# johanngerberding/voxelnet-pytorch

Hardware: AMD Instinct MI355X
Metric: point-clouds/sec fwd+bwd, KITTI car voxel grid, batch=2 (higher is better)
Workload: dtype bf16; 1 GPU; KITTI car config (voxel 0.2x0.2x0.4 m, grid 10x400x352, T=35), batch=2 per GPU, fwd+bwd train step (BASELINE configs[1]); global_batch=2, points_per_frame=19861, parallelism=dp1, launch_mode=eager+native-executor+one-call-step

## Files before the change

### include/voxelnet_hip.h

```cpp
#ifndef VOXELNET_HIP_H
#define VOXELNET_HIP_H

#include <stddef.h>
#include <stdint.h>

#ifdef __cplusplus
extern "C" {
#endif

#define VN_OK 0
#define VN_EINVAL (-1)
#define VN_EUNSUPPORTED (-2)
#define VN_EWORKSPACE (-3)

typedef enum { VN_F32 = 0, VN_BF16 = 1,
               VN_F32X3 = 2,
               VN_F32X3S = 3 } vnDtype;

typedef void *vnStream;

int vn_abi_version(void);
const char *vn_build_info(void);
const char *vn_build_id(void);

typedef struct {
    int32_t D, H, W;
    float vz, vy, vx;
    float ox, oy, oz;
    int32_t T;
} vnGrid;

size_t vn_voxelize_workspace_bytes(int64_t n_points, const vnGrid *grid);

int vn_voxelize_index(const float *points , int64_t n_points,
                      const vnGrid *grid, void *workspace, size_t workspace_bytes,
                      int32_t *k_out, vnStream stream);

int vn_voxelize_gather(const float *points, int64_t n_points, const vnGrid *grid,
                       void *workspace, size_t workspace_bytes, int64_t K,
                       int64_t batch_index, int32_t coord_cols,
                       float *feature , int64_t *coord ,
                       int64_t *number , const int32_t *k_dev, vnStream stream);

size_t vn_voxelize_host_workspace_bytes(int64_t n_points, const vnGrid *grid);
int vn_voxelize_host_index(const float *points , int64_t n_points, const vnGrid *grid,
                           void *workspace , size_t workspace_bytes, int64_t *k_out);
int vn_voxelize_host_gather(const float *points, int64_t n_points, const vnGrid *grid, const void *workspace,
                            size_t workspace_bytes, int64_t K, int64_t batch_index, int32_t coord_cols,
                            float *feature , int64_t *coord ,
                            int64_t *number );

typedef struct {
    const float *w1, *b1, *g1, *be1; float *rm1, *rv1;
    const float *w2, *b2, *g2, *be2; float *rm2, *rv2;
} vnVfeWeights;
typedef struct {
    float *dw1, *db1, *dg1, *dbe1, *dw2, *db2, *dg2, *dbe2;
} vnVfeGrads;

size_t vn_vfe_workspace_bytes(int64_t K, int32_t T);
int vn_vfe_fwd(const float *feature , int64_t K, int32_t T, const vnVfeWeights *w,
               int32_t training, float momentum, float eps, float *voxelwise ,
               float *stats , void *workspace, size_t workspace_bytes, vnStream stream);
int vn_vfe_fwd_rows(const float *feature, int64_t K, int32_t T, const vnVfeWeights *w, int32_t training, float momentum,
                    float eps, float *voxelwise, void *rows_bf16, float *stats, void *workspace, size_t workspace_bytes,
                    vnStream stream);
int vn_vfe_bwd(const float *feature, int64_t K, int32_t T, const vnVfeWeights *w, const float *stats,
               const float *d_voxelwise, const vnVfeGrads *g, void *workspace,
               size_t workspace_bytes, int32_t workspace_is_forwards, vnStream stream);

size_t vn_vfe_layer_workspace_bytes(int64_t K, int32_t T, int32_t cin, int32_t units);
int vn_vfe_layer_fwd(const float *inputs , const uint8_t *mask , int64_t K, int32_t T,
                     int32_t cin, int32_t units, const float *weight, const float *bias, const float *gamma,
                     const float *beta, float *running_mean, float *running_var, int32_t training, float momentum,
                     float eps, float *out , void *workspace, size_t workspace_bytes, vnStream stream);
int vn_vfe_layer_bwd(const float *inputs, const uint8_t *mask, const float *d_out , int64_t K,
                     int32_t T, int32_t cin, int32_t units, const float *weight, int32_t training, float *d_inputs,
                     float *d_weight, float *d_bias, float *d_gamma, float *d_beta, void *workspace,
                     size_t workspace_bytes, vnStream stream);

int vn_scatter_dense_fwd(const float *voxelwise , const int64_t *coord ,
                         int64_t K, int32_t C, int32_t B, int32_t D, int32_t H, int32_t W,
                         void *dense, vnDtype dense_dtype, int32_t dense_channels,
                         int32_t split, vnStream stream);
int vn_scatter_dense_update(const float *voxelwise , const int64_t *coord, int64_t K,
                            int32_t C, int32_t B, int32_t D, int32_t H, int32_t W, void *dense,
                            vnDtype dense_dtype, int32_t dense_channels, int32_t split, vnStream stream);

int vn_scatter_dense_bwd(const void *d_dense, vnDtype dtype, const int64_t *coord,
                         int64_t K, int32_t C, int32_t B, int32_t D, int32_t H, int32_t W,
                         float *d_voxelwise , vnStream stream);

typedef struct {
    int32_t dtype;
    int32_t B;
    int32_t Ds, Hs, Ws;
    int32_t Dr, Hr, Wr;
    int32_t Cs;
    int32_t src_wrap;
    int32_t Cr;
    int32_t kD, kH, kW;
    int32_t mulD, mulH, mulW;
    int32_t tmulD, tmulH, tmulW;
    int32_t padD, padH, padW;
    int32_t divD, divH, divW;
    int64_t src_sB, src_sD, src_sH, src_sW;
    int64_t out_sB, out_sD, out_sH, out_sW;
} vnConv;

int64_t vn_conv_stats_slab_rows(const vnConv *geom);
int vn_conv_gather_gemm(const void *src, const void *w_packed ,
                        const float *bias , void *out, vnDtype out_dtype,
                        const vnConv *geom, int32_t accumulate, float *stats_slab,
                        vnStream stream);
int32_t vn_conv_plan_id(const vnConv *geom);

size_t vn_conv_wgrad_workspace_bytes(const vnConv *geom, int32_t split, int64_t n_rows);
int vn_conv_wgrad(const void *src , const void *rows , float *dw_packed,
                  const vnConv *geom, int32_t split, void *workspace, size_t workspace_bytes,
                  vnStream stream);
int32_t vn_conv_wgrad_plan_id(const vnConv *geom, int32_t split, int64_t n_rows);
int vn_conv_wgrad_partials(const void *src, const void *rows, const vnConv *geom, int32_t split,
                           const int64_t *row_list, int64_t n_rows, void *workspace,
                           size_t workspace_bytes, int32_t *chunks, vnStream stream);
int vn_conv_wgrad_partials_split_pass(const void *src, const void *rows, const vnConv *geom, int32_t pass, void *workspace,
                                      size_t workspace_bytes, int32_t *chunks, vnStream stream);

int vn_conv_dgrad_bn_bwd(const void *src, const void *w_packed, void *out, vnDtype out_dtype, const vnConv *geom,
                         const void *bn_y, vnDtype bn_y_dtype, const float *bn_stats, float *slab, vnStream stream);
int vn_conv_gather_gemm_rows(const void *src, const void *w_packed, const float *bias, void *out,
                             vnDtype out_dtype, const vnConv *geom, const int64_t *row_list,
                             int64_t row_cap, const int32_t *row_count, int32_t out_linear,
                             float *stats_slab, vnStream stream);
int vn_conv_wgrad_rows(const void *src, const void *rows, float *dw_packed, const vnConv *geom,
                       const int64_t *row_list, int64_t n_rows, void *workspace, size_t workspace_bytes,
                       vnStream stream);
int vn_conv_wgrad_partials_counted(const void *src, const void *rows, const vnConv *geom, const int64_t *row_list,
                                   int64_t row_cap, const int32_t *row_count, void *workspace, size_t workspace_bytes,
                                   int32_t *chunks, vnStream stream);
size_t vn_active_sites_workspace_bytes(const vnConv *geom);
int vn_active_sites(const int64_t *coord, int64_t K, const vnConv *geom, void *workspace,
                    size_t workspace_bytes, int64_t *list, int64_t cap, int32_t *count, vnStream stream);
int vn_voxel_index_grid(const int64_t *coord, int64_t K, int32_t B, int32_t D, int32_t H, int32_t W,
                        int32_t *grid , vnStream stream);
int64_t vn_rulebook_slab_rows(int64_t cap);
int vn_rulebook_combine(const float *P, const int32_t *index_grid, const int64_t *list, int64_t cap,
                        const int32_t *count, const vnConv *geom, const float *bias, void *y,
                        vnDtype y_dtype, float *stats_slab, vnStream stream);
int vn_fill_rows(void *y, vnDtype dtype, int64_t M, int32_t C, int64_t stride, const float *values,
// ... 487 lines not shown
```

### voxelnet-pytorch_amd/csrc/vfe.hip

```cpp
#include "common.h"

namespace {

constexpr int C1 = 16, C2 = 64, CIN = 7;
constexpr int ST1 = 0, ST2 = 4 * C1;
constexpr int STATS_FLOATS = 4 * C1 + 4 * C2;
constexpr int TS = 65;
constexpr int NW = 2, NT = NW * 64;
constexpr int VFE_BLOCKS_MAX = 1024;
constexpr int V_AGG1 = 0, V_AM1 = 16, V_DAG1 = 32;
template <bool B2> constexpr int sv_u() { return B2 ? 48 : 16; }
template <bool B2> constexpr int sv_stride() { return B2 ? 113 : 81; }
constexpr int V_U = sv_u<true>(), V_S = V_U, SV = sv_stride<true>();
constexpr int SLAB_P1 = 64, SLAB_P2 = 2 * C2, SLAB_B1 = 2 * C2;
constexpr int SLAB_B2 = C2 + C2 * 32 + 64;
constexpr int SLAB_B3 = 128;

#ifdef VFE_TRACE
__device__ unsigned long long *g_vfe_trace;
__device__ int g_vfe_trace_kernel;
__shared__ int vfe_tr_item_s[8];
__shared__ int vfe_tr_on;
#define VFE_TR_KERNEL(id)                                                                                              \
    if (threadIdx.x == 0) vfe_tr_on = g_vfe_trace != nullptr && g_vfe_trace_kernel == (id);                            \
// ... 365 lines not shown
constexpr int PART_CHUNK = 4096;

constexpr int NCLS = 4;
__device__ __forceinline__ void classify16(const uint4 &q, int64_t v0, int64_t K, int c[NCLS]) {
    const uint32_t w[4] = {q.x, q.y, q.z, q.w};
#pragma unroll
    for (int j = 0; j < 16; ++j) {
        const int r = (w[j >> 2] >> (8 * (j & 3))) & 255;
        const bool in = v0 + j < K;
        c[0] += in && r <= 8; c[1] += in && r > 8 && r <= 16; c[2] += in && r > 16 && r <= 32; c[3] += in && r > 32;
    }
}

__global__ void __launch_bounds__(256) k_vfe_partition(const uint8_t *__restrict__ rows, int64_t K, int32_t *__restrict__ list,
                                                       int32_t *__restrict__ counts) {
    VN_PRIO_MAIN();
    __shared__ int red[4][3 * NCLS];
    const int tid = threadIdx.x, lane = tid & 63, wave = tid >> 6;
    const int64_t n16 = (K + 15) >> 4, mine = (int64_t)blockIdx.x * (PART_CHUNK / 16);
    int before[NCLS] = {0, 0, 0, 0}, total[NCLS] = {0, 0, 0, 0};
    for (int64_t i = tid; i < n16; i += 256) {
        int c[NCLS] = {0, 0, 0, 0};
        classify16(*reinterpret_cast<const uint4 *>(rows + i * 16), i * 16, K, c);
#pragma unroll
        for (int k = 0; k < NCLS; ++k) { total[k] += c[k]; before[k] += i < mine ? c[k] : 0; }
    }
    const int64_t v0 = (mine + tid) * 16;
    int c[NCLS] = {0, 0, 0, 0};
    uint4 q = make_uint4(0, 0, 0, 0);
    if (v0 < K) {
        q = *reinterpret_cast<const uint4 *>(rows + v0);
        classify16(q, v0, K, c);
    }
    int inc[NCLS];
#pragma unroll
    for (int k = 0; k < NCLS; ++k) {
        int x = c[k], t = total[k], bf = before[k];
#pragma unroll
        for (int o = 1; o < 64; o <<= 1) {
            const int y = __shfl_up(x, o, 64);
            if (lane >= o) x += y;
            t += __shfl_xor(t, o, 64);
            bf += __shfl_xor(bf, o, 64);
        }
        inc[k] = x;
        if (lane == 63) red[wave][k] = x;
        if (lane == 0) { red[wave][NCLS + k] = t; red[wave][2 * NCLS + k] = bf; }
    }
    __syncthreads();
    int pos[NCLS], tot[NCLS];
#pragma unroll
    for (int k = 0; k < NCLS; ++k) {
        int base = 0, t = 0, bf = 0;
        for (int w = 0; w < 4; ++w) {
            if (w < wave) base += red[w][k];
            t += red[w][NCLS + k];
            bf += red[w][2 * NCLS + k];
        }
        tot[k] = t;
        pos[k] = bf + base + inc[k] - c[k];
    }
    pos[1] += tot[0];
    pos[2] += tot[0] + tot[1];
    pos[3] += tot[0] + tot[1] + tot[2];
    if (v0 < K) {
        const uint32_t w[4] = {q.x, q.y, q.z, q.w};
#pragma unroll
        for (int j = 0; j < 16; ++j) {
            const int r = (w[j >> 2] >> (8 * (j & 3))) & 255;
            if (v0 + j < K) {
                if (r <= 8) list[pos[0]++] = (int32_t)(v0 + j);
                else if (r <= 16) list[pos[1]++] = (int32_t)(v0 + j);
                else if (r <= 32) list[pos[2]++] = (int32_t)(v0 + j);
                else list[pos[3]++] = (int32_t)(v0 + j);
            }
        }
    }
    if (blockIdx.x == 0 && tid == 0) { counts[0] = tot[0]; counts[1] = tot[1]; counts[2] = tot[2]; counts[3] = tot[3]; }
}

template <int G>
__device__ __forceinline__ void p2_item(const float *__restrict__ feature, int T, const WorkList &wk, int first, int n,
                                        int item, const float *wl, const float *stats, const WaveLds &L, int lane,
                                        const FwdRegs &F, float &s1, float &s2) {
    int v, r, s, j; float wgt;
    item_lane<G>(wk, first, n, item, T, lane, v, r, s, j, wgt);
    float x[CIN], m, h1[C1], p1[C1];
    load_row(feature, v, T, j, j < r, x, m);
    forward_to_h2<G, false, false>(wl, stats, L, lane, v, r, s, j, x, m, F, h1, p1);
    L.mk[lane] = wgt;
    __builtin_amdgcn_wave_barrier();
    for (int t = 0; t < 64; ++t) {
        const float h = L.tile[t * TS + lane], wh = L.mk[t] * h;
        s1 += wh;
        s2 = fmaf(wh, h, s2);
    }
    __builtin_amdgcn_wave_barrier();
}

__global__ void __launch_bounds__(NT) __attribute__((amdgpu_waves_per_eu(2, 2))) k_vfe_p2(const float *__restrict__ feature, int T, VfeParams P, WorkList wk,
                                               const float *__restrict__ stats, float *__restrict__ slabs) {
    VN_PRIO_MAIN();
    extern __shared__ __attribute__((aligned(16))) float smem[];
    const int lane = threadIdx.x & 63, wave = threadIdx.x >> 6;
    VFE_TR_KERNEL(2)
    float *wl = smem;
    load_weights_lds(P, wl, smem + WL_SIZE);
    const WaveLds L = carve_lds<false>(smem + WL_SIZE, wave);
    const Items it = load_items(wk);
    FwdRegs F;
    load_fwd_regs(P, smem + WL_SIZE, lane, F);
    __syncthreads();
    float s1 = 0.f, s2 = 0.f;
#define BODY_P2(G, first, n, item) p2_item<G>(feature, T, wk, first, n, item, wl, stats, L, lane, F, s1, s2);
    VFE_FOR_ITEMS(it, BODY_P2)
#undef BODY_P2
    __syncthreads();
    float vals[2] = {s1, s2};
    slab_write(smem, vals, 2, lane, wave, slabs + (size_t)blockIdx.x * SLAB_P2);
}

template <int G>
__device__ __forceinline__ void p3_item(const float *__restrict__ feature, int T, const WorkList &wk, int first, int n,
                                        int item, const float *wl, const float *stats, const WaveLds &L, int lane,
                                        const FwdRegs &F, float mean2, float S2, float be2,
                                        float *__restrict__ voxelwise, bf16_t *__restrict__ rows16) {
    constexpr int R = 64 / G;
    int v, r, s, j; float wgt;
    item_lane<G>(wk, first, n, item, T, lane, v, r, s, j, wgt);
    float x[CIN], m, h1[C1], p1[C1];
    load_row(feature, v, T, j, j < r, x, m);
    forward_to_h2<G, false, false>(wl, stats, L, lane, v, r, s, j, x, m, F, h1, p1);
    for (int ts = 0; ts < G; ++ts) {
        const int tv = uni(L.sid[ts]), tr = uni(L.sid[8 + ts]);
        if (tv < 0) continue;
        float agg = -INFINITY, vlo = -INFINITY, anym = 0.f, allm = 1.f;
        for (int t = 0; t < tr; ++t) {
            const float p = fmaf(S2, L.tile[(ts * R + t) * TS + lane] - mean2, be2);
            const float mk = L.mk[ts * R + t];
            agg = fmaxf(agg, p);
            vlo = fmaxf(vlo, p * mk);
            anym = fmaxf(anym, mk);
            allm = fminf(allm, mk);
        }
        float vhi = agg * anym;
        if (anym != allm) vhi = fmaxf(agg, 0.f);
        voxelwise[(int64_t)tv * 128 + lane] = vlo;
        voxelwise[(int64_t)tv * 128 + 64 + lane] = vhi;
        if (rows16) {
            rows16[(int64_t)tv * 128 + lane] = (bf16_t)vlo;
            rows16[(int64_t)tv * 128 + 64 + lane] = (bf16_t)vhi;
        }
    }
    __builtin_amdgcn_wave_barrier();
}

__global__ void __launch_bounds__(NT) __attribute__((amdgpu_waves_per_eu(2, 2))) k_vfe_p3(const float *__restrict__ feature, int T, VfeParams P, WorkList wk,
                                               const float *__restrict__ stats, float *__restrict__ voxelwise,
                                               bf16_t *__restrict__ rows16) {
    VN_PRIO_MAIN();
    extern __shared__ __attribute__((aligned(16))) float smem[];
    const int lane = threadIdx.x & 63, wave = threadIdx.x >> 6;
    VFE_TR_KERNEL(3)
    float *wl = smem;
    load_weights_lds(P, wl, smem + WL_SIZE);
    const WaveLds L = carve_lds<false>(smem + WL_SIZE, wave);
    const Items it = load_items(wk);
    FwdRegs F;
    load_fwd_regs(P, smem + WL_SIZE, lane, F);
    __syncthreads();
    const float mean2 = stats[ST2 + lane], S2 = stats[ST2 + 2 * C2 + lane], be2 = stats[ST2 + 3 * C2 + lane];
#define BODY_P3(G, first, n, item) p3_item<G>(feature, T, wk, first, n, item, wl, stats, L, lane, F, mean2, S2, be2, voxelwise, rows16);
    VFE_FOR_ITEMS(it, BODY_P3)
#undef BODY_P3
}

__device__ __forceinline__ void slab_pair_sum(const float *__restrict__ slabs, int nslabs, int stride, int off, int C,
                                              int c, double &o1, double &o2) {
    __shared__ double r1[4], r2[4];
    double s1 = 0.0, s2 = 0.0;
    for (int b = threadIdx.x; b < nslabs; b += 256) {
        s1 += slabs[(size_t)b * stride + off + c];
        s2 += slabs[(size_t)b * stride + off + C + c];
    }
#pragma unroll
    for (int o = 32; o > 0; o >>= 1) {
        s1 += __shfl_xor(s1, o, 64);
        s2 += __shfl_xor(s2, o, 64);
    }
    if ((threadIdx.x & 63) == 0) { r1[threadIdx.x >> 6] = s1; r2[threadIdx.x >> 6] = s2; }
    __syncthreads();
    o1 = (r1[0] + r1[1]) + (r1[2] + r1[3]);
    o2 = (r2[0] + r2[1]) + (r2[2] + r2[3]);
}

__global__ void __launch_bounds__(256) k_vfe_finalize(const float *__restrict__ slabs, int nslabs, int slab_stride, int C,
                                                      int64_t rows,
                                                      const float *__restrict__ gamma, const float *__restrict__ beta,
                                                      float *running_mean, float *running_var, int training,
                                                      float momentum, float eps, float *__restrict__ st) {
    VN_PRIO_MAIN();
    const int c = blockIdx.x;
    double mean, var;
    float p_gamma = 0.f, p_beta = 0.f, p_rm = 0.f, p_rv = 0.f;
    if (threadIdx.x == 0) { p_gamma = gamma[c]; p_beta = beta[c]; p_rm = running_mean[c]; p_rv = running_var[c]; }
    if (training) {
        double s1, s2;
        slab_pair_sum(slabs, nslabs, slab_stride, 0, C, c, s1, s2);
        const double n = (double)rows;
        mean = s1 / n;
        var = s2 / n - mean * mean;
        if (var < 0.0) var = 0.0;
        if (threadIdx.x == 0) {
            running_mean[c] = (float)((1.0 - momentum) * p_rm + momentum * mean);
            const double unb = n > 1.0 ? var * n / (n - 1.0) : var;
            running_var[c] = (float)((1.0 - momentum) * p_rv + momentum * unb);
        }
    } else {
        mean = p_rm;
        var = p_rv;
    }
    if (threadIdx.x == 0) {
        const float invstd = (float)(1.0 / sqrt(var + (double)eps));
        st[c] = (float)mean;
        st[C + c] = invstd;
        st[2 * C + c] = p_gamma * invstd;
        st[3 * C + c] = p_beta;
    }
}

template <int R>
__device__ __forceinline__ void impulses(const WaveLds &L, int row0, int tr, int lane, float mean2, float S2, float be2,
                                         float dlo, float dhi, int &r1, float &g1, int &r2, float &g2, float &xh1,
                                         float &xh2, float inv2) {
    float agg = -INFINITY, vlo = -INFINITY;
    r1 = 0; r2 = 0;
    float h_r1 = 0.f, h_r2 = 0.f, mk_r1 = 0.f;
#pragma unroll
    for (int t0 = 0; t0 < R; t0 += 8) {
        if (R > 16 && t0 >= tr) break;
        float h[8];
#pragma unroll
        for (int u = 0; u < 8; ++u) h[u] = L.tile[(row0 + t0 + u) * TS + lane];
        const f32x4_t ma = *reinterpret_cast<const f32x4_t *>(L.mk + row0 + t0), mb = *reinterpret_cast<const f32x4_t *>(L.mk + row0 + t0 + 4);
        const float mk[8] = {ma[0], ma[1], ma[2], ma[3], mb[0], mb[1], mb[2], mb[3]};
#pragma unroll
        for (int u = 0; u < 8; ++u) {
            const int t = t0 + u;
            const float p = fmaf(S2, h[u] - mean2, be2);
            const float pm = p * mk[u];
            const bool c2 = t < tr && p > agg, c1 = t < tr && pm > vlo;
            agg = c2 ? p : agg; r2 = c2 ? t : r2; h_r2 = c2 ? h[u] : h_r2;
            vlo = c1 ? pm : vlo; r1 = c1 ? t : r1; h_r1 = c1 ? h[u] : h_r1; mk_r1 = c1 ? mk[u] : mk_r1;
        }
    }
    float best = -INFINITY, mk_ap = 0.f;
#pragma unroll
// ... 288 lines not shown
    const int lane = threadIdx.x & 63, wave = threadIdx.x >> 6;
    VFE_TR_KERNEL(-1)
    const Items it = load_items(wk);
    float acc[C1 * CIN + C1];
#pragma unroll
    for (int e = 0; e < C1 * CIN + C1; ++e) acc[e] = 0.f;
#define BODY_B3(G, first, n, item)                                                                                   \
    {                                                                                                                \
        int v, r, s, j; float wgt;                                                                                   \
        item_lane<G>(wk, first, n, item, T, lane, v, r, s, j, wgt);                                                  \
        const bool active = j < r;                                                                                   \
        float x[CIN], m, h1[C1];                                                                                     \
        load_row(feature, v, T, j, active, x, m);                                                                    \
        layer1(P, x, h1);                                                                                            \
        if (active) {                                                                                                \
            const float *src = dp1_ws + ((int64_t)v * T + j) * C1;                                                   \
            _Pragma("unroll") for (int i = 0; i < C1; i += 4) {                                                      \
                const float4 d = *reinterpret_cast<const float4 *>(src + i);                                         \
                const float dd[4] = {d.x, d.y, d.z, d.w};                                                            \
                _Pragma("unroll") for (int q = 0; q < 4; ++q) {                                                      \
                    const int o = i + q;                                                                             \
                    const float dh = fmaf(coef1[o], dd[q], wgt * fmaf(coef1[C1 + o], h1[o] - stats[ST1 + o], coef1[2 * C1 + o])); \
                    const float da = h1[o] > 0.f ? dh : 0.f;                                                         \
                    acc[C1 * CIN + o] += da;                                                                         \
                    _Pragma("unroll") for (int k = 0; k < CIN; ++k) acc[o * CIN + k] = fmaf(da, x[k], acc[o * CIN + k]); \
                }                                                                                                    \
            }                                                                                                        \
        }                                                                                                            \
    }
    VFE_FOR_ITEMS(it, BODY_B3)
#undef BODY_B3
    lane_sums_to_slab(acc, smem, lane, wave, slabs + (size_t)blockIdx.x * SLAB_B3);
}

struct ReduceJobs {
    const float *slabs[4];
    float *out[4];
    int stride[4], off[4], n[4], first[5], nslabs[4];
};
constexpr int RED_E = 16, RED_G = 64;
__global__ void __launch_bounds__(RED_E * RED_G) k_vfe_reduce_multi(const ReduceJobs J) {
    VN_PRIO_MAIN();
    int j = 0;
#pragma unroll
    for (int q = 1; q < 4; ++q)
        if ((int)blockIdx.x >= J.first[q]) j = q;
    const float *slabs = J.slabs[0];
    float *out = J.out[0];
    int stride = J.stride[0], off = J.off[0], n = J.n[0], first = J.first[0], nslabs = J.nslabs[0];
#pragma unroll
    for (int q = 1; q < 4; ++q)
        if (j == q) {
            slabs = J.slabs[q]; out = J.out[q]; stride = J.stride[q]; off = J.off[q]; n = J.n[q]; first = J.first[q];
            nslabs = J.nslabs[q];
        }
    __shared__ double red[RED_G][RED_E + 1];
    const int e = threadIdx.x & (RED_E - 1), g = threadIdx.x / RED_E;
    const int i = ((int)blockIdx.x - first) * RED_E + e;
    double s = 0.0;
    if (i < n) {
        for (int b0 = g; b0 < nslabs; b0 += RED_G * 16) {
            float x[16];
#pragma unroll
            for (int u = 0; u < 16; ++u) {
                const int b = b0 + RED_G * u;
                x[u] = b < nslabs ? slabs[(size_t)b * stride + off + i] : 0.f;
            }
#pragma unroll
            for (int u = 0; u < 16; ++u) s += x[u];
        }
    }
    red[g][e] = s;
    __syncthreads();
    if (threadIdx.x < RED_E && i < n) {
        double t = 0.0;
        for (int q = 0; q < RED_G; ++q) t += red[q][threadIdx.x];
        out[i] = (float)t;
    }
}

struct Plan {
    int blocks, blocks_b2;
    size_t lds_small, lds_full, lds_b2;
    size_t off_slabs, off_slabs3, off_coef, off_rows, off_list, off_counts, off_dp1, bytes;
};

Plan make_plan(int64_t K, int T) {
    Plan p{};
    int64_t b = vn_ceil_div(K, 2 * NW);
    if (b < 1) b = 1;
    if (b > VFE_BLOCKS_MAX) b = VFE_BLOCKS_MAX;
    p.blocks = (int)b;
    p.blocks_b2 = b > 512 ? 512 : (int)b;
    p.lds_small = (size_t)NW * 32 * TS * sizeof(float);
    p.lds_full = (size_t)(WL_SIZE + NW * wave_floats<false>()) * sizeof(float);
    static_assert(W2_STAGE <= NW * wave_floats<false>(), "the W2 staging area must fit the per-wave areas");
    size_t full = (size_t)(WL_END + NW * wave_floats<true>()) * sizeof(float);
    const size_t red = (size_t)NW * 32 * 64 * sizeof(float);
    if (full < red) full = red;
    p.lds_b2 = full;
    size_t off = 0;
    auto take = [&](size_t bytes) { size_t r = off; off += vn_align(bytes); return r; };
    const size_t k1 = (size_t)(K > 0 ? K : 1);
    p.off_slabs = take((size_t)VFE_BLOCKS_MAX * SLAB_B2 * sizeof(float));
    p.off_slabs3 = take((size_t)VFE_BLOCKS_MAX * SLAB_B3 * sizeof(float));
    p.off_coef = take((size_t)(3 * C1 + 3 * C2) * sizeof(float));
    p.off_rows = take(k1);
    p.off_list = take(k1 * sizeof(int32_t));
    p.off_counts = take(4 * sizeof(int32_t));
    p.off_dp1 = take(k1 * T * C1 * sizeof(float));
    p.bytes = off;
    return p;
}

int set_lds_attrs() {
    static const hipError_t st = [] {
        const void *fns[] = {reinterpret_cast<const void *>(&k_vfe_p2),
                             reinterpret_cast<const void *>(&k_vfe_p3), reinterpret_cast<const void *>(&k_vfe_b1),
                             reinterpret_cast<const void *>(&k_vfe_b2), reinterpret_cast<const void *>(&k_vfe_b3)};
        for (const void *f : fns) {
#ifdef VFE_TRACE
            const int max_dyn = 160 * 1024 - 1024;
#else
            const int max_dyn = 160 * 1024;
#endif
            const hipError_t e = hipFuncSetAttribute(f, hipFuncAttributeMaxDynamicSharedMemorySize, max_dyn);
            if (e != hipSuccess) return e;
        }
        return hipSuccess;
    }();
    return (int)st;
}

int build_worklist(const float *feature, int64_t K, int T, char *ws, const Plan &pl, hipStream_t st, WorkList *wk,
                   const VfeParams *P = nullptr, float *p1_slabs = nullptr, int *p1_blocks = nullptr) {
    uint8_t *rows = reinterpret_cast<uint8_t *>(ws + pl.off_rows);
    int32_t *list = reinterpret_cast<int32_t *>(ws + pl.off_list);
    int32_t *counts = reinterpret_cast<int32_t *>(ws + pl.off_counts);
    if (p1_slabs) {
        int64_t b = vn_ceil_div(K, 4 * RP_WAVES);
        if (b > VFE_BLOCKS_MAX) b = VFE_BLOCKS_MAX;
        *p1_blocks = (int)b;
        k_vfe_rows_p1<<<(unsigned)b, 64 * RP_WAVES, 0, st>>>(feature, K, T, rows, *P, p1_slabs);
    } else {
        k_vfe_rows<<<(unsigned)vn_ceil_div(K, 4), 256, 0, st>>>(feature, K, T, rows);
    }
    VN_LAUNCH_STATUS();
    k_vfe_partition<<<(unsigned)vn_ceil_div(K, PART_CHUNK), 256, 0, st>>>(rows, K, list, counts);
    VN_LAUNCH_STATUS();
    *wk = WorkList{rows, list, counts};
    return VN_OK;
}

}

#ifdef VFE_TRACE
extern "C" int vn_debug_vfe_trace(void *buf, int kernel) {
    VN_HIP(hipMemcpyToSymbol(HIP_SYMBOL(g_vfe_trace), &buf, sizeof(buf)));
    VN_HIP(hipMemcpyToSymbol(HIP_SYMBOL(g_vfe_trace_kernel), &kernel, sizeof(kernel)));
    return VN_OK;
}
#endif

extern "C" size_t vn_vfe_workspace_bytes(int64_t K, int32_t T) {
    if (K < 0 || K >= (1ll << 31) / 64 || T <= 0 || T > 64) return 0;
    return make_plan(K, T).bytes;
}

static int vfe_fwd(const float *feature, int64_t K, int32_t T, const vnVfeWeights *w, int32_t training, float momentum,
                   float eps, float *voxelwise, void *rows_bf16, float *stats, void *workspace, size_t workspace_bytes,
                   vnStream stream) {
    VN_CHECK_ARG(w && stats && workspace && K >= 0 && K < (1ll << 31) / 64 && T > 0 && T <= 64);
    VN_CHECK_ARG(w->w1 && w->b1 && w->g1 && w->be1 && w->rm1 && w->rv1 && w->w2 && w->b2 && w->g2 && w->be2 && w->rm2 &&
                 w->rv2);
    const Plan pl = make_plan(K, T);
    if (workspace_bytes < pl.bytes) return VN_EWORKSPACE;
    hipStream_t st = vn_stream(stream);
    char *ws = static_cast<char *>(workspace);
    float *slabs = reinterpret_cast<float *>(ws + pl.off_slabs);
    const VfeParams P{w->w1, w->b1, w->w2, w->b2};
    if (const int e = set_lds_attrs()) return e;
    const int64_t rows = K * T;
    WorkList wk{};
    int p1_blocks = 0;
    if (K > 0) {
        VN_CHECK_ARG(feature && voxelwise);
        if (const int e = training ? build_worklist(feature, K, T, ws, pl, st, &wk, &P, slabs, &p1_blocks)
                                   : build_worklist(feature, K, T, ws, pl, st, &wk))
            return e;
    }
    if (training) {
        VN_CHECK_ARG(K > 0);
        k_vfe_finalize<<<C1, 256, 0, st>>>(slabs, p1_blocks, SLAB_P1, C1, rows, w->g1, w->be1, w->rm1, w->rv1, 1, momentum,
                                         eps, stats + ST1);
        VN_LAUNCH_STATUS();
        k_vfe_p2<<<pl.blocks, NT, pl.lds_full, st>>>(feature, T, P, wk, stats, slabs);
        VN_LAUNCH_STATUS();
        k_vfe_finalize<<<C2, 256, 0, st>>>(slabs, pl.blocks, SLAB_P2, C2, rows, w->g2, w->be2, w->rm2, w->rv2, 1, momentum,
                                         eps, stats + ST2);
        VN_LAUNCH_STATUS();
    } else {
        k_vfe_finalize<<<C1, 256, 0, st>>>(nullptr, 0, 0, C1, rows, w->g1, w->be1, w->rm1, w->rv1, 0, momentum, eps, stats + ST1);
        VN_LAUNCH_STATUS();
        k_vfe_finalize<<<C2, 256, 0, st>>>(nullptr, 0, 0, C2, rows, w->g2, w->be2, w->rm2, w->rv2, 0, momentum, eps, stats + ST2);
        VN_LAUNCH_STATUS();
    }
    if (K == 0) return VN_OK;
    k_vfe_p3<<<pl.blocks, NT, pl.lds_full, st>>>(feature, T, P, wk, stats, voxelwise, static_cast<bf16_t *>(rows_bf16));
    VN_LAUNCH_STATUS();
    return VN_OK;
}

extern "C" int vn_vfe_fwd(const float *feature, int64_t K, int32_t T, const vnVfeWeights *w, int32_t training,
                          float momentum, float eps, float *voxelwise, float *stats, void *workspace,
                          size_t workspace_bytes, vnStream stream) {
    return vfe_fwd(feature, K, T, w, training, momentum, eps, voxelwise, nullptr, stats, workspace, workspace_bytes, stream);
}

extern "C" int vn_vfe_fwd_rows(const float *feature, int64_t K, int32_t T, const vnVfeWeights *w, int32_t training,
                               float momentum, float eps, float *voxelwise, void *rows_bf16, float *stats, void *workspace,
                               size_t workspace_bytes, vnStream stream) {
    VN_CHECK_ARG(rows_bf16 || K == 0);
    return vfe_fwd(feature, K, T, w, training, momentum, eps, voxelwise, rows_bf16, stats, workspace, workspace_bytes, stream);
}

extern "C" int vn_vfe_bwd(const float *feature, int64_t K, int32_t T, const vnVfeWeights *w, const float *stats,
                          const float *d_voxelwise, const vnVfeGrads *g, void *workspace, size_t workspace_bytes,
                          int32_t workspace_is_forwards, vnStream stream) {
    VN_CHECK_ARG(feature && w && stats && d_voxelwise && g && workspace && K > 0 && K < (1ll << 31) / 64 && T > 0 && T <= 64);
    VN_CHECK_ARG(g->dw1 && g->db1 && g->dg1 && g->dbe1 && g->dw2 && g->db2 && g->dg2 && g->dbe2);
    const Plan pl = make_plan(K, T);
    if (workspace_bytes < pl.bytes) return VN_EWORKSPACE;
    const int eval = (workspace_is_forwards >> 1) & 1;
    workspace_is_forwards &= 1;
    hipStream_t st = vn_stream(stream);
    char *ws = static_cast<char *>(workspace);
    float *slabs = reinterpret_cast<float *>(ws + pl.off_slabs);
    float *coef1 = reinterpret_cast<float *>(ws + pl.off_coef);
    float *coef2 = coef1 + 3 * C1;
    float *dp1 = reinterpret_cast<float *>(ws + pl.off_dp1);
    const VfeParams P{w->w1, w->b1, w->w2, w->b2};
    if (const int e = set_lds_attrs()) return e;
    const int64_t rows = K * T;
    WorkList wk{};
    if (workspace_is_forwards) {
        wk = WorkList{reinterpret_cast<const uint8_t *>(ws + pl.off_rows), reinterpret_cast<const int32_t *>(ws + pl.off_list),
                      reinterpret_cast<const int32_t *>(ws + pl.off_counts)};
    } else if (const int e = build_worklist(feature, K, T, ws, pl, st, &wk)) {
        return e;
    }
    k_vfe_b1<<<pl.blocks, NT, pl.lds_full, st>>>(feature, T, P, wk, stats, d_voxelwise, slabs);
    VN_LAUNCH_STATUS();
    k_vfe_bn_bwd_finalize<<<C2, 256, 0, st>>>(slabs, pl.blocks, SLAB_B1, 0, C2, rows, w->g2, stats + ST2, coef2, g->dg2, g->dbe2, eval);
    VN_LAUNCH_STATUS();
    k_vfe_b2<<<pl.blocks_b2, NT, pl.lds_b2, st>>>(feature, T, P, wk, stats, d_voxelwise, coef2, dp1, slabs);
    VN_LAUNCH_STATUS();
    k_vfe_bn_bwd_finalize<<<C1, 256, 0, st>>>(slabs, pl.blocks_b2, SLAB_B2, C2 + C2 * 32, C1, rows, w->g1, stats + ST1, coef1,
                                            g->dg1, g->dbe1, eval);
    VN_LAUNCH_STATUS();
    float *slabs3 = reinterpret_cast<float *>(ws + pl.off_slabs3);
    k_vfe_b3<<<pl.blocks, NT, pl.lds_small, st>>>(feature, T, P, wk, stats, coef1, dp1, slabs3);
    VN_LAUNCH_STATUS();
    {
        ReduceJobs J{};
        const float *sl[4] = {slabs, slabs, slabs3, slabs3};
        float *out[4] = {g->db2, g->dw2, g->dw1, g->db1};
        const int stride[4] = {SLAB_B2, SLAB_B2, SLAB_B3, SLAB_B3}, off[4] = {0, C2, 0, C1 * CIN};
        const int n[4] = {C2, C2 * 32, C1 * CIN, C1};
        int first = 0;
        for (int j = 0; j < 4; ++j) {
            J.slabs[j] = sl[j]; J.out[j] = out[j]; J.stride[j] = stride[j]; J.off[j] = off[j]; J.n[j] = n[j];
            J.nslabs[j] = j < 2 ? pl.blocks_b2 : pl.blocks;
            J.first[j] = first;
            first += (n[j] + RED_E - 1) / RED_E;
        }
        J.first[4] = first;
        k_vfe_reduce_multi<<<first, RED_E * RED_G, 0, st>>>(J);
        VN_LAUNCH_STATUS();
    }
    return VN_OK;
}
```

### voxelnet-pytorch_amd/voxelnet_amd/_lib.py

```python
import ctypes
import os

import torch

_HERE = os.path.dirname(os.path.abspath(__file__))
LIB_PATH = os.environ.get("VN_LIB_PATH") or os.path.join(_HERE, "lib", "libvoxelnet_hip.so")

c_i32, c_i64, c_f32, c_vp, c_sz = ctypes.c_int32, ctypes.c_int64, ctypes.c_float, ctypes.c_void_p, ctypes.c_size_t

VN_F32, VN_BF16 = 0, 1
VN_F32X3S = 3


class VnGrid(ctypes.Structure):
    _fields_ = [("D", c_i32), ("H", c_i32), ("W", c_i32),
                ("vz", c_f32), ("vy", c_f32), ("vx", c_f32),
                ("ox", c_f32), ("oy", c_f32), ("oz", c_f32), ("T", c_i32)]


class VnConv(ctypes.Structure):
    _fields_ = [(n, c_i32) for n in (
        "dtype", "B", "Ds", "Hs", "Ws", "Dr", "Hr", "Wr", "Cs", "src_wrap", "Cr", "kD", "kH", "kW",
        "mulD", "mulH", "mulW", "tmulD", "tmulH", "tmulW", "padD", "padH", "padW",
        "divD", "divH", "divW")] + [(n, c_i64) for n in (
# ... 82 lines not shown
class VnLossSpec(ctypes.Structure):
    _fields_ = [("cls_kind", c_i32), ("yaw_sin", c_i32), ("focal_alpha", c_f32), ("focal_gamma", c_f32)]


class VnStep(ctypes.Structure):
    _fields_ = [("feature", c_vp), ("coord", c_vp), ("K", c_i64), ("T", c_i32), ("bn_momentum", c_f32), ("bn_eps", c_f32),
                ("vfe", VnVfeWeights), ("vfe_grads", VnVfeGrads), ("vfe_ws", c_vp), ("vfe_ws_bytes", c_sz),
                ("voxelwise", c_vp), ("vfe_stats", c_vp), ("vw_rows", c_vp), ("d_voxelwise", c_vp),
                ("prob_w", c_vp), ("prob_b", c_vp), ("reg_w", c_vp), ("reg_b", c_vp), ("heads_w", c_vp), ("heads_b", c_vp),
                ("d_heads_w", c_vp), ("d_heads_b", c_vp), ("layers", c_vp), ("grads", c_vp), ("ws", c_vp), ("ws_bytes", c_sz),
                ("prob", c_vp), ("reg", c_vp), ("d_prob", c_vp), ("d_reg", c_vp), ("pos", c_vp), ("neg", c_vp),
                ("targets", c_vp), ("targets_stream", c_vp), ("alpha", c_f32), ("beta", c_f32), ("sigma", c_f32),
                ("loss_ws", c_vp), ("loss_ws_bytes", c_sz), ("loss5", c_vp), ("g_loss", c_vp), ("chunks", c_vp),
                ("n_chunks", c_i32), ("max_norm", c_f32), ("lr", c_f32), ("scale_grads", c_i32), ("opt_ws", c_vp),
                ("opt_ws_bytes", c_sz), ("total_norm", c_vp), ("bn_counters", c_vp), ("n_bn_counters", c_i32), ("stream", c_vp),
                ("side_stream", c_vp), ("loss_spec", VnLossSpec)]


class VnAugmentBox(ctypes.Structure):
    _fields_ = [("lo", c_f32 * 3), ("hi", c_f32 * 3), ("tx", ctypes.c_double), ("ty", ctypes.c_double), ("tz", ctypes.c_double),
                ("c", ctypes.c_double), ("s", ctypes.c_double)]


VN_AUGMENT_BOXES, VN_AUGMENT_ROTATE, VN_AUGMENT_SCALE = 0, 1, 2
VN_AUGMENT_MAX_BOXES = 128


class VnObjectMove(ctypes.Structure):
    _fields_ = [(n, ctypes.c_double) for n in ("x", "y", "z0", "z1", "hl", "hw", "c", "s", "tx", "ty", "tz", "rc", "rs")] + \
               [("pad", ctypes.c_double * 3)]


class VnAffine(ctypes.Structure):
    _fields_ = [(n, ctypes.c_double) for n in ("a00", "a01", "a10", "a11", "sz", "bx", "by", "bz")]


class VnGtBox(ctypes.Structure):
    _fields_ = [(n, ctypes.c_double) for n in ("x", "y", "z0", "z1", "hl", "hw", "c", "s")]


VN_GT_MAX_BOXES = 128
VN_EVAL_BEV, VN_EVAL_3D = 0, 1
VN_EVAL_MAX_TOPK, VN_EVAL_MAX_DIFF = 32, 8
VN_EVAL_BBOX, VN_EVAL_MAX_DC, VN_EVAL_IMAGE_ROW = 2, 64, 12
VN_NMS_STANDUP, VN_NMS_ROTATED = 0, 1
VN_DETECT_MAX_PRE, VN_PREDICT_MAX_TOPK = 4096, 64
VN_DETECT_FLAT, VN_DETECT_SITE = 0, 1
VN_ASSIGN_STANDUP, VN_ASSIGN_ROTATED = 1, 2


_P = ctypes.POINTER
SIGNATURES = {
    "vn_abi_version": (c_i32, []),
    "vn_build_info": (ctypes.c_char_p, []),
    "vn_build_id": (ctypes.c_char_p, []),
    "vn_voxelize_workspace_bytes": (c_sz, [c_i64, _P(VnGrid)]),
    "vn_voxelize_index": (c_i32, [c_vp, c_i64, _P(VnGrid), c_vp, c_sz, c_vp, c_vp]),
    "vn_voxelize_gather": (c_i32, [c_vp, c_i64, _P(VnGrid), c_vp, c_sz, c_i64, c_i64, c_i32, c_vp, c_vp, c_vp, c_vp, c_vp]),
    "vn_voxelize_host_workspace_bytes": (c_sz, [c_i64, _P(VnGrid)]),
    "vn_voxelize_host_index": (c_i32, [c_vp, c_i64, _P(VnGrid), c_vp, c_sz, _P(c_i64)]),
    "vn_voxelize_host_gather": (c_i32, [c_vp, c_i64, _P(VnGrid), c_vp, c_sz, c_i64, c_i64, c_i32, c_vp, c_vp, c_vp]),
    "vn_vfe_layer_workspace_bytes": (c_sz, [c_i64, c_i32, c_i32, c_i32]),
    "vn_vfe_layer_fwd": (c_i32, [c_vp, c_vp, c_i64, c_i32, c_i32, c_i32, c_vp, c_vp, c_vp, c_vp, c_vp, c_vp, c_i32, c_f32, c_f32,
                                 c_vp, c_vp, c_sz, c_vp]),
    "vn_vfe_layer_bwd": (c_i32, [c_vp, c_vp, c_vp, c_i64, c_i32, c_i32, c_i32, c_vp, c_i32, c_vp, c_vp, c_vp, c_vp, c_vp, c_vp,
                                 c_sz, c_vp]),
    "vn_fov_crop_workspace_bytes": (c_sz, [c_i64]),
    "vn_fov_crop": (c_i32, [c_vp, c_i64, c_vp, c_vp, c_vp, c_i32, c_i32, c_vp, c_vp, c_vp, c_vp, c_sz, c_vp]),
    "vn_augment_points": (c_i32, [c_vp, c_i64, c_i32, c_vp, c_i32, ctypes.c_double, ctypes.c_double, c_f32, c_vp, c_vp]),
    "vn_augment_compose": (c_i32, [c_vp, c_i64, c_vp, c_i32, c_vp, c_vp, c_vp]),
    "vn_points_in_boxes": (c_i32, [c_vp, c_i64, c_vp, c_i32, c_vp, c_vp, c_vp]),
    "vn_gt_paste_workspace_bytes": (c_sz, [c_i64]),
    "vn_gt_paste": (c_i32, [c_vp, c_i64, c_vp, c_i32, c_vp, c_i64, c_vp, c_i64, c_vp, c_vp, c_sz, c_vp]),
    "vn_permute_points": (c_i32, [c_vp, c_i64, c_vp, c_vp, c_vp]),
    "vn_shuffle_points": (c_i32, [c_vp, c_i64, c_vp, c_vp, c_vp]),
    "vn_comm_rccl_version": (c_i32, []),
    "vn_comm_unique_id": (c_i32, [c_vp]),
    "vn_comm_create": (c_i32, [_P(c_vp), c_vp, c_i32, c_i32]),
    "vn_comm_destroy": (c_i32, [c_vp]),
    "vn_allreduce_bucket": (c_i32, [c_vp, c_vp, c_i64, c_f32, c_vp]),
    "vn_vfe_workspace_bytes": (c_sz, [c_i64, c_i32]),
    "vn_vfe_fwd": (c_i32, [c_vp, c_i64, c_i32, _P(VnVfeWeights), c_i32, c_f32, c_f32, c_vp, c_vp, c_vp, c_sz, c_vp]),
    "vn_vfe_fwd_rows": (c_i32, [c_vp, c_i64, c_i32, _P(VnVfeWeights), c_i32, c_f32, c_f32, c_vp, c_vp, c_vp, c_vp, c_sz, c_vp]),
    "vn_vfe_bwd": (c_i32, [c_vp, c_i64, c_i32, _P(VnVfeWeights), c_vp, c_vp, _P(VnVfeGrads), c_vp, c_sz, c_i32, c_vp]),
    "vn_scatter_dense_fwd": (c_i32, [c_vp, c_vp, c_i64, c_i32, c_i32, c_i32, c_i32, c_i32, c_vp, c_i32, c_i32,
                                     c_i32, c_vp]),
    "vn_scatter_dense_update": (c_i32, [c_vp, c_vp, c_i64, c_i32, c_i32, c_i32, c_i32, c_i32, c_vp, c_i32, c_i32,
                                        c_i32, c_vp]),
    "vn_scatter_dense_bwd": (c_i32, [c_vp, c_i32, c_vp, c_i64, c_i32, c_i32, c_i32, c_i32, c_i32, c_vp, c_vp]),
    "vn_conv_gather_gemm": (c_i32, [c_vp, c_vp, c_vp, c_vp, c_i32, _P(VnConv), c_i32, c_vp, c_vp]),
    "vn_net_workspace_bytes": (c_sz, [_P(VnNetConfig), c_i64]),
    "vn_net_tensor_info": (c_i32, [_P(VnNetConfig), c_i64, c_i32, c_i32, _P(VnNetTensorInfo)]),
    "vn_net_create": (c_i32, [_P(c_vp)]),
    "vn_net_destroy": (c_i32, [c_vp]),
    "vn_net_step": (c_i32, [c_vp, _P(VnNetConfig), _P(VnStep)]),
    "vn_net_timing_begin": (c_i32, [c_vp, c_i32]),
    "vn_net_timing_read": (c_i32, [c_vp, c_vp, c_i32, _P(c_i32)]),
    "vn_net_forward": (c_i32, [c_vp, _P(VnNetConfig), _P(VnLayerParams), c_vp, c_vp, c_vp, c_vp, c_vp, c_i64, c_vp, c_sz, c_vp,
                               c_vp, c_vp, c_vp]),
    "vn_net_wait_bucket": (c_i32, [c_vp, c_i32, c_vp]),
    "vn_net_prepare": (c_i32, [c_vp, _P(VnNetConfig), _P(VnLayerParams), c_vp, c_vp, c_i64, c_vp, c_sz, c_vp]),
    "vn_voxel_index_grid": (c_i32, [c_vp, c_i64, c_i32, c_i32, c_i32, c_i32, c_vp, c_vp]),
    "vn_rulebook_slab_rows": (c_i64, [c_i64]),
    "vn_rulebook_combine": (c_i32, [c_vp, c_vp, c_vp, c_i64, c_vp, _P(VnConv), c_vp, c_vp, c_i32, c_vp, c_vp]),
    "vn_net_backward": (c_i32, [c_vp, _P(VnNetConfig), _P(VnLayerParams), c_vp, c_vp, c_vp, c_vp, c_vp, c_vp, c_vp, c_i64,
                                c_vp, c_sz, _P(VnLayerGrads), c_vp, c_vp, c_vp, c_i32, c_i32, c_vp, c_vp]),
    "vn_conv_stats_slab_rows": (c_i64, [_P(VnConv)]),
    "vn_conv_plan_id": (c_i32, [_P(VnConv)]),
    "vn_conv_wgrad_plan_id": (c_i32, [_P(VnConv), c_i32, c_i64]),
    "vn_bn_finalize_slab": (c_i32, [c_vp, c_i64, c_i64, c_i32, c_vp, c_vp, c_vp, c_vp, c_vp, c_f32, c_f32, c_vp, c_vp]),
    "vn_conv_wgrad_workspace_bytes": (c_sz, [_P(VnConv), c_i32, c_i64]),
    "vn_conv_wgrad": (c_i32, [c_vp, c_vp, c_vp, _P(VnConv), c_i32, c_vp, c_sz, c_vp]),
    "vn_conv_dgrad_bn_bwd": (c_i32, [c_vp, c_vp, c_vp, c_i32, _P(VnConv), c_vp, c_i32, c_vp, c_vp, c_vp]),
    "vn_conv_gather_gemm_rows": (c_i32, [c_vp, c_vp, c_vp, c_vp, c_i32, _P(VnConv), c_vp, c_i64, c_vp, c_i32, c_vp, c_vp]),
    "vn_conv_wgrad_partials": (c_i32, [c_vp, c_vp, _P(VnConv), c_i32, c_vp, c_i64, c_vp, c_sz, c_vp, c_vp]),
    "vn_conv_wgrad_rows": (c_i32, [c_vp, c_vp, c_vp, _P(VnConv), c_vp, c_i64, c_vp, c_sz, c_vp]),
    "vn_conv_wgrad_partials_split_pass": (c_i32, [c_vp, c_vp, _P(VnConv), c_i32, c_vp, c_sz, c_vp, c_vp]),
    "vn_active_sites_workspace_bytes": (c_sz, [_P(VnConv)]),
    "vn_active_sites": (c_i32, [c_vp, c_i64, _P(VnConv), c_vp, c_sz, c_vp, c_i64, c_vp, c_vp]),
    "vn_fill_rows": (c_i32, [c_vp, c_i32, c_i64, c_i32, c_i64, c_vp, c_vp]),
    "vn_pack_weight": (c_i32, [c_vp, c_i32, c_i32, c_i32, c_i32, c_i32, c_i32, c_vp, c_i32, c_vp]),
    "vn_unpack_wgrad": (c_i32, [c_vp, c_i32, c_i32, c_i32, c_i32, c_i32, c_vp, c_vp]),
    "vn_bn_stats": (c_i32, [c_vp, c_i32, c_i64, c_i32, c_i64, c_i32, c_vp, c_vp, c_vp]),
    "vn_bn_finalize": (c_i32, [c_vp, c_i64, c_i32, c_i32, c_vp, c_vp, c_vp, c_vp, c_vp, c_i32, c_f32, c_f32, c_vp,
                               c_vp]),
    "vn_bn_apply": (c_i32, [c_vp, c_i32, c_i64, c_i64, c_i32, c_vp, c_i32, c_vp, c_i32, c_i64, c_i64, c_vp]),
    "vn_bn_bwd_reduce": (c_i32, [c_vp, c_i32, c_i64, c_vp, c_i32, c_i64, c_i64, c_i32, c_vp, c_i32, c_vp, c_vp]),
    "vn_bn_bwd_finalize": (c_i32, [c_vp, c_i64, c_i32, c_i32, c_vp, c_vp, c_vp, c_vp, c_vp, c_vp]),
    "vn_bn_bwd_slab_rows": (c_i64, [c_i64, c_i32]),
    "vn_bn_bwd_reduce_slab": (c_i32, [c_vp, c_i32, c_i64, c_vp, c_i32, c_i64, c_i64, c_i32, c_vp, c_i32, c_vp, c_vp]),
    "vn_bn_bwd_finalize_slab": (c_i32, [c_vp, c_i64, c_i64, c_i32, c_vp, c_vp, c_vp, c_vp, c_vp, c_vp]),
    "vn_bn_bwd_apply": (c_i32, [c_vp, c_i32, c_i64, c_vp, c_i32, c_i64, c_i64, c_i32, c_vp, c_vp, c_i32, c_vp,
                                c_i32, c_i64, c_i64, c_vp]),
    "vn_bn_apply_bev": (c_i32, [c_vp, c_i32, c_i64, c_i32, c_i64, c_vp, c_i32, c_vp, c_i32, c_i64, c_vp]),
    "vn_bn_bwd_reduce_slab_bev": (c_i32, [c_vp, c_i32, c_i64, c_vp, c_i32, c_i64, c_i32, c_i64, c_vp, c_i32, c_vp, c_vp]),
    "vn_bn_bwd_apply_bev": (c_i32, [c_vp, c_i32, c_i64, c_vp, c_i32, c_i64, c_i32, c_i64, c_vp, c_vp, c_i32, c_vp, c_i32, c_vp]),
    "vn_bn_apply_flagged": (c_i32, [c_vp, c_i32, c_i64, c_i64, c_i32, c_vp, c_i32, c_vp, c_i32, c_i64, c_vp, c_vp, c_vp]),
    "vn_bn_bwd_reduce_slab_flagged": (c_i32, [c_vp, c_i32, c_i64, c_vp, c_i32, c_i64, c_i64, c_i32, c_vp, c_i32, c_vp, c_vp, c_vp,
                                              c_vp]),
    "vn_bn_bwd_apply_list": (c_i32, [c_vp, c_i32, c_vp, c_i32, c_i32, c_i32, c_i32, c_i32, c_vp, c_vp, c_i32, c_vp, c_i32, c_vp,
                                     c_vp, c_i64, c_vp]),
    "vn_bn_bwd_list_slab_rows": (c_i64, [c_i64, c_i32]),
    "vn_bn_bwd_reduce_list": (c_i32, [c_vp, c_i32, c_vp, c_i32, c_i32, c_i32, c_i32, c_i32, c_vp, c_i32, c_vp, c_vp, c_vp, c_i64, c_vp]),
    "vn_bn_bwd_finalize_list": (c_i32, [c_vp, c_i64, c_i64, c_i32, c_vp, c_vp, c_vp, c_vp, c_i32, c_i32, c_vp, c_vp, c_vp, c_vp]),
    "vn_bn_bwd_apply_list_rows": (c_i32, [c_vp, c_i32, c_vp, c_i32, c_i32, c_i32, c_i32, c_i32, c_vp, c_vp, c_i32, c_vp, c_i32,
                                          c_vp, c_vp, c_i64, c_vp]),
    "vn_dgrad_total_workspace_bytes": (c_sz, [c_i32]),
    "vn_dgrad_total": (c_i32, [c_vp, c_i32, c_i32, c_i32, c_i32, c_i32, c_i32, c_i32, c_i32, c_vp, c_i32, c_vp, c_sz, c_vp, c_vp]),
    "vn_box_col_sums": (c_i32, [c_vp, c_i32, c_i32, c_i32, c_i32, c_i32, c_i32, c_vp, c_sz, c_vp]),
    "vn_act_delta_rows": (c_i32, [c_vp, c_i32, c_i32, c_i32, c_i32, c_i32, c_vp, c_vp, c_i32, c_i32, c_vp, c_vp, c_i64, c_vp, c_i32,
                                  c_vp]),
    "vn_wgrad_const_add": (c_i32, [c_vp, c_vp, c_sz, c_i32, c_i32, c_i32, c_vp, c_vp, c_i32, c_i32, c_i32, c_vp]),
    "vn_conv_wgrad_partials_counted": (c_i32, [c_vp, c_vp, _P(VnConv), c_vp, c_i64, c_vp, c_vp, c_sz, c_vp, c_vp]),
    "vn_bn_bwd_apply_flagged": (c_i32, [c_vp, c_i32, c_i64, c_vp, c_i32, c_i64, c_i64, c_i32, c_vp, c_vp, c_i32, c_vp, c_i32,
                                        c_i64, c_vp, c_vp]),
    "vn_nchw_to_rows": (c_i32, [c_vp, c_i32, c_i32, c_i64, c_vp, c_i32, c_i64, c_i64, c_vp]),
    "vn_rows_to_nchw": (c_i32, [c_vp, c_i32, c_i64, c_i32, c_i32, c_i64, c_vp, c_i32, c_vp]),
    "vn_cast_rows": (c_i32, [c_vp, c_i32, c_i64, c_i64, c_i32, c_vp, c_i32, c_i64, c_i64, c_vp]),
    "vn_col_sums_workspace_bytes": (c_sz, [c_i64, c_i32]),
    "vn_col_sums": (c_i32, [c_vp, c_i32, c_i64, c_i64, c_i32, c_vp, c_vp, c_sz, c_vp]),
    "vn_heads_to_nchw": (c_i32, [c_vp, c_i32, c_i64, c_vp, c_vp, c_vp]),
    "vn_heads_fwd": (c_i32, [c_vp, c_i64, c_vp, c_vp, c_i32, c_i64, c_vp, c_vp, c_vp]),
    "vn_heads_dgrad": (c_i32, [c_vp, c_i64, c_vp, c_vp, c_i64, c_i64, c_vp]),
    "vn_heads_dgrad_f32": (c_i32, [c_vp, c_i64, c_vp, c_vp, c_i32, c_i64, c_i64, c_vp]),
    "vn_heads_bwd": (c_i32, [c_vp, c_vp, c_vp, c_i32, c_i64, c_vp, c_i32, c_i64, c_i32, c_vp]),
    "vn_pack_weights_batch": (c_i32, [c_vp, c_i32, c_vp]),
# ... 152 lines not shown
```

Before: 571.5 point-clouds/s.

## Store per-voxel h2 max/min in VFE pass 2 to skip pass-3 recompute

Pass 2 of the VFE forward now also records, for each voxel and channel, the max and min of the pre-BN second-layer activations over the unmasked points, plus a flag for whether any masked points exist. In training mode a new lightweight elementwise kernel rebuilds the BN+ReLU+maxpool output from these extrema, using the sign of the BN scale to pick max or min. This replaces the full pass-3 recompute of both layers per point. The trade is an extra K×128-float workspace buffer and more stores in pass 2. Correctness depends on BN being monotone per channel, and the masked rows are assumed to produce relu(b2).

Result: no change. 572.2 point-clouds/s, median of 3 (+0.1%).

```diff
diff --git a/include/voxelnet_hip.h b/include/voxelnet_hip.h
--- a/include/voxelnet_hip.h
+++ b/include/voxelnet_hip.h
@@ -65,6 +65,9 @@
 int vn_vfe_fwd_rows(const float *feature, int64_t K, int32_t T, const vnVfeWeights *w, int32_t training, float momentum,
                     float eps, float *voxelwise, void *rows_bf16, float *stats, void *workspace, size_t workspace_bytes,
                     vnStream stream);
+int vn_vfe_fwd_recompute(const float *feature, int64_t K, int32_t T, const vnVfeWeights *w, int32_t training, float momentum,
+                         float eps, float *voxelwise, void *rows_bf16, float *stats, void *workspace, size_t workspace_bytes,
+                         vnStream stream);
 int vn_vfe_bwd(const float *feature, int64_t K, int32_t T, const vnVfeWeights *w, const float *stats,
                const float *d_voxelwise, const vnVfeGrads *g, void *workspace,
                size_t workspace_bytes, int32_t workspace_is_forwards, vnStream stream);
diff --git a/voxelnet-pytorch_amd/csrc/vfe.hip b/voxelnet-pytorch_amd/csrc/vfe.hip
--- a/voxelnet-pytorch_amd/csrc/vfe.hip
+++ b/voxelnet-pytorch_amd/csrc/vfe.hip
@@ -471,24 +471,40 @@
 template <int G>
 __device__ __forceinline__ void p2_item(const float *__restrict__ feature, int T, const WorkList &wk, int first, int n,
                                         int item, const float *wl, const float *stats, const WaveLds &L, int lane,
-                                        const FwdRegs &F, float &s1, float &s2) {
+                                        const FwdRegs &F, float &s1, float &s2, float *__restrict__ hext) {
+    constexpr int R = 64 / G;
     int v, r, s, j; float wgt;
     item_lane<G>(wk, first, n, item, T, lane, v, r, s, j, wgt);
     float x[CIN], m, h1[C1], p1[C1];
     load_row(feature, v, T, j, j < r, x, m);
     forward_to_h2<G, false, false>(wl, stats, L, lane, v, r, s, j, x, m, F, h1, p1);
-    L.mk[lane] = wgt;
+    L.mk[lane] = m != 0.f ? wgt : -wgt;
     __builtin_amdgcn_wave_barrier();
-    for (int t = 0; t < 64; ++t) {
-        const float h = L.tile[t * TS + lane], wh = L.mk[t] * h;
-        s1 += wh;
-        s2 = fmaf(wh, h, s2);
+#pragma unroll 1
+    for (int ts = 0; ts < G; ++ts) {
+        float mx = -INFINITY, mn = INFINITY;
+        bool masked = false;
+#pragma unroll 8
+        for (int t = ts * R; t < ts * R + R; ++t) {
+            const float e = L.mk[t], h = L.tile[t * TS + lane], wh = fabsf(e) * h;
+            s1 += wh;
+            s2 = fmaf(wh, h, s2);
+            mx = e > 0.f ? fmaxf(mx, h) : mx;
+            mn = e > 0.f ? fminf(mn, h) : mn;
+            masked |= e < 0.f;
+        }
+        const int tv = uni(L.sid[ts]);
+        if (tv >= 0) {
+            hext[(int64_t)tv * 128 + lane] = mx;
+            hext[(int64_t)tv * 128 + 64 + lane] = __uint_as_float(__float_as_uint(mn) | (masked ? 0x80000000u : 0u));
+        }
     }
     __builtin_amdgcn_wave_barrier();
 }
 
 __global__ void __launch_bounds__(NT) __attribute__((amdgpu_waves_per_eu(2, 2))) k_vfe_p2(const float *__restrict__ feature, int T, VfeParams P, WorkList wk,
-                                               const float *__restrict__ stats, float *__restrict__ slabs) {
+                                               const float *__restrict__ stats, float *__restrict__ slabs,
+                                               float *__restrict__ hext) {
     VN_PRIO_MAIN();
     extern __shared__ __attribute__((aligned(16))) float smem[];
     const int lane = threadIdx.x & 63, wave = threadIdx.x >> 6;
@@ -501,7 +517,7 @@
     load_fwd_regs(P, smem + WL_SIZE, lane, F);
     __syncthreads();
     float s1 = 0.f, s2 = 0.f;
-#define BODY_P2(G, first, n, item) p2_item<G>(feature, T, wk, first, n, item, wl, stats, L, lane, F, s1, s2);
+#define BODY_P2(G, first, n, item) p2_item<G>(feature, T, wk, first, n, item, wl, stats, L, lane, F, s1, s2, hext);
     VFE_FOR_ITEMS(it, BODY_P2)
 #undef BODY_P2
     __syncthreads();
@@ -562,6 +578,39 @@
 #define BODY_P3(G, first, n, item) p3_item<G>(feature, T, wk, first, n, item, wl, stats, L, lane, F, mean2, S2, be2, voxelwise, rows16);
     VFE_FOR_ITEMS(it, BODY_P3)
 #undef BODY_P3
+}
+
+__global__ void __launch_bounds__(256) k_vfe_p3e(int64_t K, const float *__restrict__ hext, const float *__restrict__ b2,
+                                                 const float *__restrict__ stats, float *__restrict__ voxelwise,
+                                                 bf16_t *__restrict__ rows16) {
+    VN_PRIO_MAIN();
+    const int64_t i = (int64_t)blockIdx.x * 256 + threadIdx.x;
+    const int64_t v = i >> 6;
+    const int c = (int)(i & 63);
+    if (v >= K) return;
+    const float mean2 = stats[ST2 + c], S2 = stats[ST2 + 2 * C2 + c], be2 = stats[ST2 + 3 * C2 + c];
+    const float hmax = hext[v * 128 + c];
+    const uint32_t mnb = __float_as_uint(hext[v * 128 + 64 + c]);
+    const bool masked = (mnb >> 31) != 0, unmasked = hmax != -INFINITY;
+    const float hmin = __uint_as_float(mnb & 0x7fffffffu);
+    const float pu = fmaf(S2, ((__float_as_uint(S2) >> 31) ? hmin : hmax) - mean2, be2);
+    const float pm = fmaf(S2, fmaxf(b2[c], 0.f) - mean2, be2);
+    float agg, vlo, vhi;
+    if (unmasked && masked) {
+        agg = fmaxf(pu, pm);
+        vlo = fmaxf(pu, pm * 0.f);
+        vhi = fmaxf(agg, 0.f);
+    } else if (unmasked) {
+        agg = pu; vlo = pu; vhi = agg;
+    } else {
+        agg = pm; vlo = pm * 0.f; vhi = agg * 0.f;
+    }
+    voxelwise[v * 128 + c] = vlo;
+    voxelwise[v * 128 + 64 + c] = vhi;
+    if (rows16) {
+        rows16[v * 128 + c] = (bf16_t)vlo;
+        rows16[v * 128 + 64 + c] = (bf16_t)vhi;
+    }
 }
 
 __device__ __forceinline__ void slab_pair_sum(const float *__restrict__ slabs, int nslabs, int stride, int off, int C,
@@ -1016,7 +1065,7 @@
 struct Plan {
     int blocks, blocks_b2;
     size_t lds_small, lds_full, lds_b2;
-    size_t off_slabs, off_slabs3, off_coef, off_rows, off_list, off_counts, off_dp1, bytes;
+    size_t off_slabs, off_slabs3, off_coef, off_rows, off_list, off_counts, off_dp1, off_hext, bytes;
 };
 
 Plan make_plan(int64_t K, int T) {
@@ -1043,6 +1092,7 @@
     p.off_list = take(k1 * sizeof(int32_t));
     p.off_counts = take(4 * sizeof(int32_t));
     p.off_dp1 = take(k1 * T * C1 * sizeof(float));
+    p.off_hext = take(k1 * 2 * C2 * sizeof(float));
     p.bytes = off;
     return p;
 }
@@ -1103,7 +1153,7 @@
 
 static int vfe_fwd(const float *feature, int64_t K, int32_t T, const vnVfeWeights *w, int32_t training, float momentum,
                    float eps, float *voxelwise, void *rows_bf16, float *stats, void *workspace, size_t workspace_bytes,
-                   vnStream stream) {
+                   bool recompute, vnStream stream) {
     VN_CHECK_ARG(w && stats && workspace && K >= 0 && K < (1ll << 31) / 64 && T > 0 && T <= 64);
     VN_CHECK_ARG(w->w1 && w->b1 && w->g1 && w->be1 && w->rm1 && w->rv1 && w->w2 && w->b2 && w->g2 && w->be2 && w->rm2 &&
                  w->rv2);
@@ -1128,7 +1178,7 @@
         k_vfe_finalize<<<C1, 256, 0, st>>>(slabs, p1_blocks, SLAB_P1, C1, rows, w->g1, w->be1, w->rm1, w->rv1, 1, momentum,
                                          eps, stats + ST1);
         VN_LAUNCH_STATUS();
-        k_vfe_p2<<<pl.blocks, NT, pl.lds_full, st>>>(feature, T, P, wk, stats, slabs);
+        k_vfe_p2<<<pl.blocks, NT, pl.lds_full, st>>>(feature, T, P, wk, stats, slabs, reinterpret_cast<float *>(ws + pl.off_hext));
         VN_LAUNCH_STATUS();
         k_vfe_finalize<<<C2, 256, 0, st>>>(slabs, pl.blocks, SLAB_P2, C2, rows, w->g2, w->be2, w->rm2, w->rv2, 1, momentum,
                                          eps, stats + ST2);
@@ -1140,7 +1190,11 @@
         VN_LAUNCH_STATUS();
     }
     if (K == 0) return VN_OK;
-    k_vfe_p3<<<pl.blocks, NT, pl.lds_full, st>>>(feature, T, P, wk, stats, voxelwise, static_cast<bf16_t *>(rows_bf16));
+    if (training && !recompute)
+        k_vfe_p3e<<<(unsigned)vn_ceil_div(K * C2, 256), 256, 0, st>>>(K, reinterpret_cast<const float *>(ws + pl.off_hext), w->b2, stats,
+                                                                   voxelwise, static_cast<bf16_t *>(rows_bf16));
+    else
+        k_vfe_p3<<<pl.blocks, NT, pl.lds_full, st>>>(feature, T, P, wk, stats, voxelwise, static_cast<bf16_t *>(rows_bf16));
     VN_LAUNCH_STATUS();
     return VN_OK;
 }
@@ -1148,14 +1202,20 @@
 extern "C" int vn_vfe_fwd(const float *feature, int64_t K, int32_t T, const vnVfeWeights *w, int32_t training,
                           float momentum, float eps, float *voxelwise, float *stats, void *workspace,
                           size_t workspace_bytes, vnStream stream) {
-    return vfe_fwd(feature, K, T, w, training, momentum, eps, voxelwise, nullptr, stats, workspace, workspace_bytes, stream);
+    return vfe_fwd(feature, K, T, w, training, momentum, eps, voxelwise, nullptr, stats, workspace, workspace_bytes, false, stream);
 }
 
 extern "C" int vn_vfe_fwd_rows(const float *feature, int64_t K, int32_t T, const vnVfeWeights *w, int32_t training,
                                float momentum, float eps, float *voxelwise, void *rows_bf16, float *stats, void *workspace,
                                size_t workspace_bytes, vnStream stream) {
     VN_CHECK_ARG(rows_bf16 || K == 0);
-    return vfe_fwd(feature, K, T, w, training, momentum, eps, voxelwise, rows_bf16, stats, workspace, workspace_bytes, stream);
+    return vfe_fwd(feature, K, T, w, training, momentum, eps, voxelwise, rows_bf16, stats, workspace, workspace_bytes, false, stream);
+}
+
+extern "C" int vn_vfe_fwd_recompute(const float *feature, int64_t K, int32_t T, const vnVfeWeights *w, int32_t training,
+                                    float momentum, float eps, float *voxelwise, void *rows_bf16, float *stats, void *workspace,
+                                    size_t workspace_bytes, vnStream stream) {
+    return vfe_fwd(feature, K, T, w, training, momentum, eps, voxelwise, rows_bf16, stats, workspace, workspace_bytes, true, stream);
 }
 
 extern "C" int vn_vfe_bwd(const float *feature, int64_t K, int32_t T, const vnVfeWeights *w, const float *stats,
diff --git a/voxelnet-pytorch_amd/voxelnet_amd/_lib.py b/voxelnet-pytorch_amd/voxelnet_amd/_lib.py
--- a/voxelnet-pytorch_amd/voxelnet_amd/_lib.py
+++ b/voxelnet-pytorch_amd/voxelnet_amd/_lib.py
@@ -188,6 +188,7 @@
     "vn_vfe_workspace_bytes": (c_sz, [c_i64, c_i32]),
     "vn_vfe_fwd": (c_i32, [c_vp, c_i64, c_i32, _P(VnVfeWeights), c_i32, c_f32, c_f32, c_vp, c_vp, c_vp, c_sz, c_vp]),
     "vn_vfe_fwd_rows": (c_i32, [c_vp, c_i64, c_i32, _P(VnVfeWeights), c_i32, c_f32, c_f32, c_vp, c_vp, c_vp, c_vp, c_sz, c_vp]),
+    "vn_vfe_fwd_recompute": (c_i32, [c_vp, c_i64, c_i32, _P(VnVfeWeights), c_i32, c_f32, c_f32, c_vp, c_vp, c_vp, c_vp, c_sz, c_vp]),
     "vn_vfe_bwd": (c_i32, [c_vp, c_i64, c_i32, _P(VnVfeWeights), c_vp, c_vp, _P(VnVfeGrads), c_vp, c_sz, c_i32, c_vp]),
     "vn_scatter_dense_fwd": (c_i32, [c_vp, c_vp, c_i64, c_i32, c_i32, c_i32, c_i32, c_i32, c_vp, c_i32, c_i32,
                                      c_i32, c_vp]),
```
